# nadult/Snail

Measured on AMD Instinct MI355X. Metric: Mrays/sec (primary), higher is better.
Workload: dtype f32; 1 GPU; BASELINE config 1: atrium (263124 tris, sponza.obj stand-in) 1920x1080 primary rays, hit records (t,u,v,triId); reflections=False, arith=host_sse, arith_tables=host CPU, packets=16x16 px = 1 wavefront, bvh_nodes=161677, bvh_depth=21, frames_in_flight=16, frames_per_launch=4, launches_in_flight=4, settle_frames=332, order_refresh=16, ranks=1, packet_order=heaviest first (node visits of an earlier frame), parallelism=single-gpu

## Files before the change

include/snail_hip_debug.h:

```cpp
#ifndef SNAIL_HIP_DEBUG_H
#define SNAIL_HIP_DEBUG_H
#include "snail_hip.h"
#ifdef __cplusplus
extern "C" {
#endif

int snail_debug_delay_dev(float microseconds, void *stream);

int snail_debug_clock_dev(float microseconds, uint64_t *d_out2, void *stream);

int snail_debug_recip_check(uint64_t out2[2]);

int snail_debug_hostsse_device_check(int fn, int threads, uint64_t *badChunks, uint32_t *firstBadChunk);

int snail_debug_dispatch_rate(int blocks, int threads, int reps, float *ms_per_launch);

int snail_debug_anyorder(SnailScene *, const float cam[13], int resx, int resy, int frames, int flags, float *ms_total);

int snail_debug_occupancy(int out[4]);

#ifdef __cplusplus
}
#endif
#endif
```

snail_amd/_lib.py:

```python
from __future__ import annotations

import ctypes as C
import os

HERE = os.path.dirname(os.path.abspath(__file__))
LIB_PATH = os.environ.get("SNAIL_LIB_PATH") or os.path.join(HERE, "libsnailhip.so")


class SnailError(RuntimeError):
    pass


_lib = None

_VP, _I, _F13 = C.c_void_p, C.c_int, C.c_void_p
SIGNATURES = {
    "snail_last_error": (C.c_char_p, []),
    "snail_device_count": (_I, []),
    "snail_tris_from_verts": (_I, [_VP, _I, _VP]),
    "snail_bvh_build": (_I, [_VP, _I, _VP, _VP, _VP, _VP]),
    "snail_scene_create": (_VP, [_VP, _I, _VP, _I, _I, _I]),
    "snail_scene_destroy": (None, [_VP]),
    "snail_scene_info": (_I, [_VP, _VP, _VP, _VP, _VP]),
    "snail_scene_flags": (_I, [_VP, _VP, _VP]),
# ... 61 lines not shown
    "snail_instances_render_whitted_dev": (_I, [_VP, _F13, _I, _I, _VP, _I, _VP, _VP, _I, _VP, _I, _VP, _VP]),
    "snail_instances_render_whitted_packets_dev": (_I, [_VP, _F13, _I, _I, _VP, _I, _VP, _I, _VP, _VP, _I, _VP, _VP, _VP]),
    "snail_instances_render_image": (_I, [_VP, _F13, _I, _I, _VP, _I, _VP, _VP, _I, _VP, _I, _VP]),
}

INSTANCES_TILES_SIGNATURES = {
    "snail_instances_shade_packets_dev": (_I, [_VP, _F13, _I, _I, _VP, _I, _VP, _I, _VP, _VP, _I, _VP, _VP, _VP, _VP]),
    "snail_instances_render_tiles": (_I, [_VP, _F13, _I, _I, _VP, _VP, _I, _VP, _I, _VP, _VP, _I, _VP, _VP, _VP]),
    "snail_instances_render_frame": (_I, [_VP, _F13, _I, _I, _VP, _I, _VP, _VP, _I, _VP, _I, _VP]),
}

INSTANCES_BUILD_SIGNATURES = {
    "snail_instances_rebuild_dev": (_I, [_VP, _VP, _VP, _I, _VP, _VP, _VP]),
    "snail_instances_read_tree": (_I, [_VP, _VP, _I, _VP, _VP, _VP, _I, _VP]),
}

BVH_FAST_SIGNATURES = {
    "snail_bvh_build_fast": (_I, [_VP, _I, _VP, _VP, _VP, _VP]),
    "snail_scene_create_fast_dev": (_VP, [_VP, _I, _I, _VP, _VP, _VP]),
    "snail_scene_rebuild_fast_dev": (_I, [_VP, _VP, _I, _VP, _VP, _VP]),
}

HEATMAP_SIGNATURES = {
    "snail_packet_stats_dev": (_I, [_VP, _F13, _I, _I, _VP, _I, _VP, _I, _I, _VP, _VP, _VP]),
    "snail_render_heat_packets_dev": (_I, [_VP, _F13, _I, _I, _VP, _I, _VP, _I, _I, _VP, _VP, _VP, _VP]),
    "snail_render_heat_tiles": (_I, [_VP, _F13, _I, _I, _VP, _VP, _I, _VP, _I, _I, _VP, _VP]),
    "snail_render_heat_image": (_I, [_VP, _F13, _I, _I, _VP, _I, _I, _VP, _I, _VP]),
    "snail_instances_packet_stats_dev": (_I, [_VP, _F13, _I, _I, _VP, _I, _VP, _I, _I, _VP, _VP, _VP]),
    "snail_instances_heat_packets_dev": (_I, [_VP, _F13, _I, _I, _VP, _I, _VP, _I, _I, _VP, _VP, _VP, _VP, _VP]),
    "snail_instances_render_heat_tiles": (_I, [_VP, _F13, _I, _I, _VP, _VP, _I, _VP, _I, _I, _VP, _VP, _VP]),
    "snail_instances_render_heat_frame": (_I, [_VP, _F13, _I, _I, _VP, _I, _I, _VP, _I, _VP]),
}

MATERIALS_SIGNATURES = {
    "snail_shtris_pack": (_I, [_VP, _VP, _VP, _VP, _I, _VP, _VP]),
    "snail_texture_size": (C.c_int64, [_I, _I, _VP]),
    "snail_texture_build": (_I, [_VP, _I, _I, _VP, C.c_int64, _VP]),
    "snail_materials_create": (_VP, [_VP, _VP, _I, _VP, _I, _VP, _I, _VP, _I]),
    "snail_materials_destroy": (None, [_VP]),
    "snail_materials_shade_packets_dev": (_I, [_VP, _F13, _I, _I, _VP, _I, _VP, _VP, _VP, _VP, _VP, _VP]),
    "snail_render_materials_dev": (_I, [_VP, _F13, _I, _I, _VP, _I, _VP, _I, _VP, _I, _VP, _VP]),
    "snail_render_materials_packets_dev": (_I, [_VP, _F13, _I, _I, _VP, _I, _VP, _I, _VP, _I, _VP, _VP, _VP]),
    "snail_render_materials_image": (_I, [_VP, _F13, _I, _I, _VP, _I, _VP, _I, _VP, _I, _VP]),
}

DEBUG_SIGNATURES = {
    "snail_debug_delay_dev": (_I, [C.c_float, _VP]),
    "snail_debug_clock_dev": (_I, [C.c_float, _VP, _VP]),
    "snail_debug_recip_check": (_I, [_VP]),
    "snail_debug_dispatch_rate": (_I, [_I, _I, _I, _VP]),
    "snail_debug_hostsse_device_check": (_I, [_I, _I, _VP, _VP]),
    "snail_debug_occupancy": (_I, [_VP]),
    "snail_debug_anyorder": (_I, [_VP, _F13, _I, _I, _I, _I, _VP]),
}
DEBUG_LIB_PATH = os.path.join(HERE, "libsnailhip_debug.so")
_dbg = None


def debug_lib():
    global _dbg
    if _dbg is None:
        if not os.path.exists(DEBUG_LIB_PATH):
            raise SnailError("workbench library %s is missing: `make -C snail_amd/csrc debug`" % DEBUG_LIB_PATH)
        L = C.CDLL(DEBUG_LIB_PATH)
        for table in (SIGNATURES, INSTANCES_SIGNATURES, INSTANCES_SHADE_SIGNATURES, INSTANCES_TILES_SIGNATURES, INSTANCES_BUILD_SIGNATURES, BVH_FAST_SIGNATURES, HEATMAP_SIGNATURES, MATERIALS_SIGNATURES, DEBUG_SIGNATURES):
            for name, (res, args) in table.items():
                fn = getattr(L, name)
                fn.restype = res
                fn.argtypes = args
        _dbg = L
    return _dbg


def lib():
    global _lib
    if _lib is None:
        if not os.path.exists(LIB_PATH):
            raise SnailError(
                "HIP extension %s is missing: run `python -c 'import __graft_entry__ as g; g.build()'` "
                "(or `make -C snail_amd/csrc`). There is no CPU fallback." % LIB_PATH)
        try:
            L = C.CDLL(LIB_PATH)
        except OSError as e:
            raise SnailError("cannot load %s: %s" % (LIB_PATH, e)) from e
        for table in (SIGNATURES, INSTANCES_SIGNATURES, INSTANCES_SHADE_SIGNATURES, INSTANCES_TILES_SIGNATURES, INSTANCES_BUILD_SIGNATURES, BVH_FAST_SIGNATURES, HEATMAP_SIGNATURES, MATERIALS_SIGNATURES):
            for name, (res, args) in table.items():
                fn = getattr(L, name)
                fn.restype = res
                fn.argtypes = args
        for name, (res, args) in DEBUG_SIGNATURES.items():
            fn = getattr(L, name, None)
            if fn is not None:
                fn.restype = res
                fn.argtypes = args
        _lib = L
    return _lib


def check(rc: int, what: str) -> None:
    if rc != 0:
        msg = lib().snail_last_error()
        raise SnailError("%s failed (status %d): %s" % (what, rc, msg.decode() if msg else "?"))


def ptr(a):
    if a is None:
# ... 5 lines not shown
```

snail_amd/csrc/snail_dev.inc:

```
namespace SNAIL_DEV_NS {

typedef unsigned long long u64;
typedef unsigned u32x4 __attribute__((ext_vector_type(4)));
typedef const __attribute__((address_space(4))) u32x4 *scalar_ptr;

struct Node {
	float bmin[3], bmax[3];
	unsigned sub;
	int aux;
};

__device__ __forceinline__ float asf(unsigned u) { return __uint_as_float(u); }
__device__ __forceinline__ float asf(int u) { return __int_as_float(u); }

typedef const __attribute__((address_space(4))) char *scalar_bytes;
__device__ __forceinline__ Node loadNode(const uint4 *nodes, int idx) {
	const unsigned off = (unsigned)idx << 5;
	scalar_ptr p = (scalar_ptr)((scalar_bytes)(unsigned long long)nodes + off);
	u32x4 a = p[0], b = p[1];
	Node n;
	n.bmin[0] = asf(a.x); n.bmin[1] = asf(a.y); n.bmin[2] = asf(a.z);
	n.bmax[0] = asf(a.w); n.bmax[1] = asf(b.x); n.bmax[2] = asf(b.y);
	n.sub = b.z; n.aux = (int)b.w;
	return n;
// ... 875 lines not shown
	" v_readlane_b32 %[cur], %[stkN], %[sp]\n v_readlane_b32 %[fl], %[stkF], %[sp]\n"                                                      \
	" s_and_b32 %[first], %[fl], 0xff\n s_lshr_b32 %[last], %[fl], 8\n"
#define SNAIL_PUSH_2W                                                                                                                      \
	" s_lshl_b32 %[off], %[last], 8\n s_or_b32 %[off], %[off], %[first]\n"                                                                 \
	" s_mov_b32 m0, %[sp]\n v_writelane_b32 %[stkN], %[fl], m0\n v_writelane_b32 %[stkF], %[off], m0\n"
#define SNAIL_COUNT " s_add_u32 %[cnt], %[cnt], 1\n"
#define SNAIL_DRAIN_SMEM " s_waitcnt lgkmcnt(0)\n"
#define SNAIL_DESCEND_ASM(PRE, ORGOPS, SLAB, TAIL, CNTPOP, CNTVISIT, NX, FX, NY, FY, NZ, FZ)                                                 \
	asm volatile(SNAIL_DRAIN_SMEM                                                                                                          \
				 "L_pop_%=:\n"                                                                                                             \
				 " s_cmp_eq_u32 %[sp], 0\n s_cbranch_scc1 L_done_%=\n"                                                                     \
				 " s_sub_u32 %[sp], %[sp], 1\n" CNTPOP                                                                                     \
				 SNAIL_POP_2W                                                                                                              \
				 " s_lshl_b32 %[off], %[cur], 5\n s_load_dwordx8 s[84:91], %[base], %[off]\n"                                              \
				 " s_sub_u32 %[width], %[last], %[first]\n"                                                                                \
				 " s_bfm_b64 exec, %[width], %[first]\n s_bitset1_b64 exec, %[last]\n"                                                     \
				 " s_waitcnt lgkmcnt(0)\n"                                                                                                 \
				 "L_visit_%=:\n" CNTVISIT                                                                                                  \
				 PRE(NX, FX, NY, FY, NZ, FZ)                                                                                               \
				 SLAB("0", NX, FX, NY, FY, NZ, FZ) TAIL("0", "s0") SLAB("1", NX, FX, NY, FY, NZ, FZ) TAIL("1", "s1")                       \
				 SLAB("2", NX, FX, NY, FY, NZ, FZ) TAIL("2", "s2") SLAB("3", NX, FX, NY, FY, NZ, FZ) TAIL("3", "s3")                       \
				 " v_max_f32 %[s2], %[s2], %[s3]\n v_max3_f32 %[s0], %[s0], %[s1], %[s2]\n"                                                \
				 " v_cmp_le_f32 vcc, 0, %[s0]\n"                                                                                           \
				 " s_and_b64 %[alive], vcc, exec\n s_cbranch_scc0 L_pop_%=\n"                                                              \
				 " s_ff1_i32_b64 %[first], %[alive]\n s_flbit_i32_b64 %[last], %[alive]\n s_xor_b32 %[last], %[last], 63\n"                \
				 " s_sub_u32 %[width], %[last], %[first]\n"                                                                                \
				 " s_bfm_b64 exec, %[width], %[first]\n s_bitset1_b64 exec, %[last]\n"                                                     \
				 " s_cmp_lt_i32 s90, 0\n s_cbranch_scc1 L_leaf_%=\n"                                                                       \
				 " s_lshr_b32 %[cur], %[sign16], s91\n s_xor_b32 %[cur], %[cur], s91\n s_bfe_u32 %[cur], %[cur], 0x10010\n"                \
				 " s_add_u32 %[fl], s90, 1\n s_sub_u32 %[fl], %[fl], %[cur]\n"                                                             \
				 " s_add_u32 %[cur], s90, %[cur]\n s_lshl_b32 %[off], %[cur], 5\n"                                                         \
				 " s_load_dwordx8 s[84:91], %[base], %[off]\n"                                                                             \
				 SNAIL_PUSH_2W                                                                                                             \
				 " s_add_u32 %[sp], %[sp], 1\n"                                                                                            \
				 " s_waitcnt lgkmcnt(0)\n s_branch L_visit_%=\n"                                                                           \
				 "L_leaf_%=:\n s_mov_b32 %[leafSub], s90\n s_mov_b32 %[leafAux], s91\n s_branch L_end_%=\n"                                \
				 "L_done_%=:\n s_mov_b32 %[leafSub], 0\n s_mov_b32 %[leafAux], 0\n"                                                        \
				 "L_end_%=:\n s_mov_b64 exec, -1\n"                                                                                        \
				 : [sp] "+s"(sp), [first] "+s"(first), [last] "+s"(last), [cnt] "+s"(cnt), [stkN] "+v"(stkN), [stkF] "+v"(stkF),           \
				   [leafSub] "=&s"(leafSub), [leafAux] "=&s"(leafAux), [cur] "=&s"(sCur), [fl] "=&s"(sFl), [off] "=&s"(sOff),              \
				   [width] "=&s"(sWidth), [rng] "=&s"(sRng), [alive] "=&s"(sAlive), [pnx] "=&v"(vt[0]), [pny] "=&v"(vt[1]),                \
				   [pnz] "=&v"(vt[2]), [pfx] "=&v"(vt[3]), [pfy] "=&v"(vt[4]), [pfz] "=&v"(vt[5]), [t0] "=&v"(vt[6]), [t1] "=&v"(vt[7]),   \
				   [t2] "=&v"(vt[8]), [t3] "=&v"(vt[9]), [t4] "=&v"(vt[10]), [t5] "=&v"(vt[11]), [s0] "=&v"(vt[12]), [s1] "=&v"(vt[13]),   \
				   [s2] "=&v"(vt[14]), [s3] "=&v"(vt[15]), [u0] "=&v"(vt[16])                                                              \
				 : [base] "s"(nodeBase), [sign16] "s"(sign16), [lane] "v"(lane), ORGOPS(), [ix0] "v"(Q.id[0][0]), [ix1] "v"(Q.id[0][1]), [ix2] "v"(Q.id[0][2]), [ix3] "v"(Q.id[0][3]),        \
				   [iy0] "v"(Q.id[1][0]), [iy1] "v"(Q.id[1][1]), [iy2] "v"(Q.id[1][2]), [iy3] "v"(Q.id[1][3]), [iz0] "v"(Q.id[2][0]),      \
				   [iz1] "v"(Q.id[2][1]), [iz2] "v"(Q.id[2][2]), [iz3] "v"(Q.id[2][3]), [d0] "v"(Q.dist[0]), [d1] "v"(Q.dist[1]),          \
				   [d2] "v"(Q.dist[2]), [d3] "v"(Q.dist[3])                                                                                \
				 : "s84", "s85", "s86", "s87", "s88", "s89", "s90", "s91", "vcc", "scc", "m0");                                            \
	              \
	asm volatile("" ::"s"(sp), "s"(first), "s"(last), "s"(cnt), "v"(stkN), "v"(stkF), "s"(leafSub), "s"(leafAux), "s"(sCur), "s"(sFl), "s"(sOff),    \
				 "s"(sWidth), "s"(sRng), "s"(sAlive), "v"(vt[0]), "v"(vt[1]), "v"(vt[2]), "v"(vt[3]), "v"(vt[4]), "v"(vt[5]), "v"(vt[6]), "v"(vt[7]), \
				 "v"(vt[8]), "v"(vt[9]), "v"(vt[10]), "v"(vt[11]), "v"(vt[12]), "v"(vt[13]), "v"(vt[14]), "v"(vt[15]), "v"(vt[16]))
#define SNAIL_MOV_REC(D0, D1, D2, D3, S0, S1, S2, S3)                                                                                       \
	" s_mov_b64 " D0 ", " S0 "\n s_mov_b64 " D1 ", " S1 "\n s_mov_b64 " D2 ", " S2 "\n s_mov_b64 " D3 ", " S3 "\n"
#define SNAIL_A_FROM_T SNAIL_MOV_REC("s[84:85]", "s[86:87]", "s[88:89]", "s[90:91]", "s[68:69]", "s[70:71]", "s[72:73]", "s[74:75]")
#define SNAIL_PF_LEAFREQ_TRI(OTHERSET) " s_bitset0_b32 %[cur], 31\n s_load_dwordx8 " OTHERSET ", %[base], %[cur]\n"
#define SNAIL_PF_LEAFREQ_SLOT0(OTHERSET) " s_max_i32 %[cur], %[cur], 0\n s_load_dwordx8 " OTHERSET ", %[base], %[cur]\n"

#define SNAIL_PF2_NEARFAR(SUB, AUX, FARX, OTHERSET, LEAFREQ)                                                                                          \
				 " s_and_b32 %[cur], " AUX ", %[sign16]\n s_cselect_b32 %[cur], 32, 0\n"                                                       \
				 " s_xor_b32 %[cur], " SUB ", %[cur]\n s_xor_b32 " FARX ", %[cur], 32\n"                                                       \
				 LEAFREQ(OTHERSET)
#define SNAIL_PF2_TAIL(X, SUB)  \
				 " v_max_f32 %[s2], %[s2], %[s3]\n v_max3_f32 %[s0], %[s0], %[s1], %[s2]\n"                                                \
				 " v_cmpx_le_f32 vcc, 0, %[s0]\n"                                                                                           \
				 " s_cbranch_execz L_fail_%=\n"                                                                                            \
				 " s_cbranch_scc1 L_leaf" X "_%=\n"
#define SNAIL_PF2_ISLEAF(SUB) " s_cmp_lt_i32 " SUB ", 0\n"
#define SNAIL_PF2_ALIVE " s_sub_u32 %[cur], %[last], %[first]\n s_bfm_b64 %[alive], %[cur], %[first]\n s_bitset1_b64 %[alive], %[last]\n"
#define SNAIL_PF2_FIRSTLAST " s_ff1_i32_b64 %[first], exec\n s_flbit_i32_b64 %[last], exec\n s_xor_b32 %[last], %[last], 63\n"
#define SNAIL_PF2_PENDING(X, OTHERSET, SUB, AUX, FARX, FARY, PRE, SLAB, TAIL, CNTVISIT, LEAFREQ, NX, FX, NY, FY, NZ, FZ)                                                   \
				 "L_visit" X "p_%=:\n"                                                                                                      \
				 " s_waitcnt lgkmcnt(0)\n"                                                 \
				 " s_load_dwordx8 s[68:75], %[base], " FARY "\n"                              \
				 CNTVISIT PRE(NX, FX, NY, FY, NZ, FZ)                                                                                        \
				 SLAB("0", NX, FX, NY, FY, NZ, FZ) TAIL("0", "s0")                                                                           \
				 SNAIL_PF2_NEARFAR(SUB, AUX, FARX, OTHERSET, LEAFREQ)                                                                        \
				 SLAB("1", NX, FX, NY, FY, NZ, FZ) TAIL("1", "s1")                                                                           \
				 SNAIL_PF2_FIRSTLAST                                                      \
				 " s_lshl_b32 %[off], %[last], 6\n s_or_b32 %[off], %[off], %[first]\n s_lshl_b32 %[off], %[off], 20\n"                    \
				 SNAIL_PF2_ALIVE                                                                                                            \
				 SLAB("2", NX, FX, NY, FY, NZ, FZ) TAIL("2", "s2")                                                                           \
				 " s_lshr_b32 %[topw], " FARY ", 5\n s_or_b32 %[topw], %[topw], %[off]\n"                                                    \
				 " v_writelane_b32 %[stkN], %[topw], m0\n s_add_u32 m0, m0, 1\n" SNAIL_PF2_ISLEAF(SUB)                                       \
				 SLAB("3", NX, FX, NY, FY, NZ, FZ) TAIL("3", "s3")                                                                           \
				 SNAIL_PF2_TAIL(X, SUB)
#define SNAIL_PF2_LEAF(X, SUB, AUX)                                                                                                         \
				 "L_leaf" X "_%=:\n" SNAIL_PF2_FIRSTLAST                                                                                    \
				 " s_bfe_u32 %[leafSub], " SUB ", 0x190006\n s_sub_u32 %[leafSub], %[leafSub], 0x80000\n s_bitset1_b32 %[leafSub], 31\n"   \
				 " s_mov_b32 %[leafAux], " AUX "\n s_waitcnt lgkmcnt(0)\n s_branch L_end_%=\n"
#define SNAIL_DESCEND_PF2X(EXTRACLOB, PREVARS, PRE, ORGOPS, SLAB, TAIL, CNTPOP, CNTVISIT, LEAFREQ, NXA, FXA, NYA, FYA, NZA, FZA, NXB, FXB, NYB, FYB, NZB, FZB)                                                  \
	asm volatile(SNAIL_DRAIN_SMEM " s_mov_b32 m0, %[sp]\n"                                                                                \
				 "L_entry_%=:\n"                                                                                                           \
				 " s_cmp_eq_u32 m0, 0\n s_cbranch_scc1 L_done_%=\n"                                                                     \
				 " s_sub_u32 %[off], m0, 1\n"                                                                                           \
				 " v_readlane_b32 %[topw], %[stkN], %[off]\n"                                                                              \
				 " s_and_b32 %[cur], %[topw], 0xfffff\n s_lshl_b32 %[off], %[cur], 5\n"                                                    \
				 " s_load_dwordx8 s[68:75], %[base], %[off]\n"                                                                             \
				 " s_bfe_u32 %[first], %[topw], 0x60014\n s_lshr_b32 %[last], %[topw], 26\n" SNAIL_PF2_ALIVE                               \
				 "L_pop_%=:\n"                             \
				 " s_sub_u32 m0, m0, 1\n" CNTPOP                                                                                     \
				 " s_mov_b64 exec, %[alive]\n"                                                                                             \
				 " s_waitcnt lgkmcnt(0)\n" SNAIL_A_FROM_T                                                                                  \
				                   \
				 " s_sub_u32 %[off], m0, 1\n s_max_i32 %[off], %[off], 0\n"   \
				 " v_readlane_b32 %[topw], %[stkN], %[off]\n"                                                                              \
				 CNTVISIT PRE(NXA, FXA, NYA, FYA, NZA, FZA)                                                                                 \
				 SLAB("0", NXA, FXA, NYA, FYA, NZA, FZA) TAIL("0", "s0")                                                          \
				 " s_and_b32 %[cur], %[topw], 0xfffff\n s_lshl_b32 %[off], %[cur], 5\n"                                                    \
				 " s_load_dwordx8 s[68:75], %[base], %[off]\n"                                                                             \
				 SLAB("1", NXA, FXA, NYA, FYA, NZA, FZA) TAIL("1", "s1")                                                          \
				 SNAIL_PF2_NEARFAR("s90", "s91", "%[fl]", "s[76:83]", LEAFREQ)                                                                       \
				 SLAB("2", NXA, FXA, NYA, FYA, NZA, FZA) TAIL("2", "s2")                                                          \
				 " s_bfe_u32 %[first], %[topw], 0x60014\n s_lshr_b32 %[last], %[topw], 26\n" SNAIL_PF2_ALIVE SNAIL_PF2_ISLEAF("s90")        \
				 SLAB("3", NXA, FXA, NYA, FYA, NZA, FZA) TAIL("3", "s3")                                                          \
				 SNAIL_PF2_TAIL("A", "s90")                                                                                                 \
				                                                                    \
				 SNAIL_PF2_PENDING("B", "s[84:91]", "s82", "s83", "%[width]", "%[fl]", PRE, SLAB, TAIL, CNTVISIT, LEAFREQ, NXB, FXB, NYB, FYB, NZB, FZB)                   \
				                                                                    \
				 SNAIL_PF2_PENDING("A", "s[76:83]", "s90", "s91", "%[fl]", "%[width]", PRE, SLAB, TAIL, CNTVISIT, LEAFREQ, NXA, FXA, NYA, FYA, NZA, FZA)                   \
				 " s_branch L_visitBp_%=\n"                                                                                                \
				 SNAIL_PF2_LEAF("A", "s90", "s91") SNAIL_PF2_LEAF("B", "s82", "s83")                                                       \
				 "L_fail_%=:\n"                                                                                                            \
				 " s_cmp_eq_u32 m0, 0\n s_cbranch_scc0 L_pop_%=\n"                                                                      \
				 "L_done_%=:\n s_mov_b32 %[leafSub], 0\n s_mov_b32 %[leafAux], 0\n s_waitcnt lgkmcnt(0)\n"                                  \
				 "L_end_%=:\n s_mov_b64 exec, -1\n s_mov_b32 %[sp], m0\n"                                                                                        \
				 : [sp] "+s"(sp), [first] "+s"(first), [last] "+s"(last), [cnt] "+s"(cnt), [stkN] "+v"(stkN), [stkF] "+v"(stkF),           \
				   [leafSub] "=&s"(leafSub), [leafAux] "=&s"(leafAux), [cur] "=&s"(sCur), [fl] "=&s"(sFl), [off] "=&s"(sOff),              \
				   [width] "=&s"(sWidth), [topw] "=&s"(sTopw), [alive] "=&s"(sAlive), PREVARS() [t0] "=&v"(vt[6]), [t1] "=&v"(vt[7]),   \
				   [t2] "=&v"(vt[8]), [t3] "=&v"(vt[9]), [t4] "=&v"(vt[10]), [t5] "=&v"(vt[11]), [s0] "=&v"(vt[12]), [s1] "=&v"(vt[13]),   \
				   [s2] "=&v"(vt[14]), [s3] "=&v"(vt[15]), [u0] "=&v"(vt[16])                                                              \
				 : [base] "s"(nodeBase), [sign16] "s"(sign16), [lane] "v"(lane), ORGOPS(), [ix0] "v"(Q.id[0][0]), [ix1] "v"(Q.id[0][1]), [ix2] "v"(Q.id[0][2]), [ix3] "v"(Q.id[0][3]),        \
				   [iy0] "v"(Q.id[1][0]), [iy1] "v"(Q.id[1][1]), [iy2] "v"(Q.id[1][2]), [iy3] "v"(Q.id[1][3]), [iz0] "v"(Q.id[2][0]),      \
				   [iz1] "v"(Q.id[2][1]), [iz2] "v"(Q.id[2][2]), [iz3] "v"(Q.id[2][3]), [d0] "v"(Q.dist[0]), [d1] "v"(Q.dist[1]),          \
				   [d2] "v"(Q.dist[2]), [d3] "v"(Q.dist[3])                                                                                \
				 : "s68", "s69", "s70", "s71", "s72", "s73", "s74", "s75", "s76", "s77", "s78", "s79", "s80", "s81", "s82", "s83", "s84", "s85", "s86", "s87", \
				   "s88", "s89", "s90", "s91", "vcc", "scc", "m0" EXTRACLOB);                                                                        \
	asm volatile("" ::"s"(sp), "s"(first), "s"(last), "s"(cnt), "v"(stkN), "v"(stkF), "s"(leafSub), "s"(leafAux), "s"(sCur), "s"(sFl), "s"(sOff),    \
				 "s"(sWidth), "s"(sTopw), "s"(sAlive), "v"(vt[6]), "v"(vt[7]), \
				 "v"(vt[8]), "v"(vt[9]), "v"(vt[10]), "v"(vt[11]), "v"(vt[12]), "v"(vt[13]), "v"(vt[14]), "v"(vt[15]), "v"(vt[16]))
#define SNAIL_PREVARS_SHARED() [pnx] "=&v"(vt[0]), [pny] "=&v"(vt[1]), [pnz] "=&v"(vt[2]), [pfx] "=&v"(vt[3]), [pfy] "=&v"(vt[4]), [pfz] "=&v"(vt[5]),
#define SNAIL_PREVARS_NONE() [pnx] "=&v"(vt[0]), [pny] "=&v"(vt[1]), [pnz] "=&v"(vt[2]), [pfx] "=&v"(vt[3]), [pfy] "=&v"(vt[4]), [pfz] "=&v"(vt[5]),
#define SNAIL_PREVARS_SNAIL_PRE_SHARED SNAIL_PREVARS_SHARED
#define SNAIL_PREVARS_SNAIL_PRE_NONE SNAIL_PREVARS_NONE
#define SNAIL_PREVARS_SNAIL_PRE_SEL SNAIL_PREVARS_NONE
#define SNAIL_PREVARS_EMPTY()
#define SNAIL_PRE_NONE_X(NX, FX, NY, FY, NZ, FZ) ""
#define SNAIL_PREVARS_SNAIL_PRE_NONE_X SNAIL_PREVARS_EMPTY
#define SNAIL_PREVARS_of(PRE) SNAIL_PREVARS_##PRE
#define SNAIL_DESCEND_PF2(PRE, ORGOPS, SLAB, TAIL, CNTPOP, CNTVISIT, LEAFREQ, NXA, FXA, NYA, FYA, NZA, FZA, NXB, FXB, NYB, FYB, NZB, FZB)                 \
	SNAIL_DESCEND_PF2X(, SNAIL_PREVARS_of(PRE), PRE, ORGOPS, SLAB, TAIL, CNTPOP, CNTVISIT, LEAFREQ, NXA, FXA, NYA, FYA, NZA, FZA, NXB, FXB, NYB, FYB, NZB, FZB)
#define SNAIL_PRE_SEL(NX, FX, NY, FY, NZ, FZ)                                                                                               \
				 " s_bitcmp1_b32 %[sign16], 8\n s_cselect_b32 s62, " FX ", " NX "\n s_cselect_b32 s65, " NX ", " FX "\n"                       \
				 " s_bitcmp1_b32 %[sign16], 9\n s_cselect_b32 s63, " FY ", " NY "\n s_cselect_b32 s66, " NY ", " FY "\n"                       \
				 " s_bitcmp1_b32 %[sign16], 10\n s_cselect_b32 s64, " FZ ", " NZ "\n s_cselect_b32 s67, " NZ ", " FZ "\n"
#define SNAIL_SLABO_SEL(L, NX, FX, NY, FY, NZ, FZ) SNAIL_SLABO_COH(L, "s62", "s65", "s63", "s66", "s64", "s67")
#define SNAIL_SEL_CLOB , "s62", "s63", "s64", "s65", "s66", "s67"
#define SNAIL_DESCEND_PF2_SEL(ORGOPS, SLAB, TAIL, CNTPOP, CNTVISIT, LEAFREQ)                                                                \
	SNAIL_DESCEND_PF2X(SNAIL_SEL_CLOB, SNAIL_PREVARS_NONE, SNAIL_PRE_SEL, ORGOPS, SLAB, TAIL, CNTPOP, CNTVISIT, LEAFREQ, "s84", "s87", "s85", "s88", "s86", "s89", "s76", "s79", "s77", "s80", "s78", "s81")
#define SNAIL_DESCEND_PF2_PLAIN(PRE, ORGOPS, SLAB, TAIL, CNTPOP, CNTVISIT, LEAFREQ) SNAIL_DESCEND_PF2(PRE, ORGOPS, SLAB, TAIL, CNTPOP, CNTVISIT, LEAFREQ, "s84", "s87", "s85", "s88", "s86", "s89", "s76", "s79", "s77", "s80", "s78", "s81")
#define SNAIL_DESCEND_PF2_OCT(PRE, ORGOPS, SLAB, TAIL, CNTPOP, CNTVISIT, LEAFREQ, OCT)                                                                                                    \
	switch(OCT) {                                                                                                                          \
	case 0: SNAIL_DESCEND_PF2(PRE, ORGOPS, SLAB, TAIL, CNTPOP, CNTVISIT, LEAFREQ, "s84", "s87", "s85", "s88", "s86", "s89", "s76", "s79", "s77", "s80", "s78", "s81"); break;            \
	case 1: SNAIL_DESCEND_PF2(PRE, ORGOPS, SLAB, TAIL, CNTPOP, CNTVISIT, LEAFREQ, "s87", "s84", "s85", "s88", "s86", "s89", "s79", "s76", "s77", "s80", "s78", "s81"); break;            \
	case 2: SNAIL_DESCEND_PF2(PRE, ORGOPS, SLAB, TAIL, CNTPOP, CNTVISIT, LEAFREQ, "s84", "s87", "s88", "s85", "s86", "s89", "s76", "s79", "s80", "s77", "s78", "s81"); break;            \
	case 3: SNAIL_DESCEND_PF2(PRE, ORGOPS, SLAB, TAIL, CNTPOP, CNTVISIT, LEAFREQ, "s87", "s84", "s88", "s85", "s86", "s89", "s79", "s76", "s80", "s77", "s78", "s81"); break;            \
	case 4: SNAIL_DESCEND_PF2(PRE, ORGOPS, SLAB, TAIL, CNTPOP, CNTVISIT, LEAFREQ, "s84", "s87", "s85", "s88", "s89", "s86", "s76", "s79", "s77", "s80", "s81", "s78"); break;            \
	case 5: SNAIL_DESCEND_PF2(PRE, ORGOPS, SLAB, TAIL, CNTPOP, CNTVISIT, LEAFREQ, "s87", "s84", "s85", "s88", "s89", "s86", "s79", "s76", "s77", "s80", "s81", "s78"); break;            \
	case 6: SNAIL_DESCEND_PF2(PRE, ORGOPS, SLAB, TAIL, CNTPOP, CNTVISIT, LEAFREQ, "s84", "s87", "s88", "s85", "s89", "s86", "s76", "s79", "s80", "s77", "s81", "s78"); break;            \
	default: SNAIL_DESCEND_PF2(PRE, ORGOPS, SLAB, TAIL, CNTPOP, CNTVISIT, LEAFREQ, "s87", "s84", "s88", "s85", "s89", "s86", "s79", "s76", "s80", "s77", "s81", "s78"); break;           \
	}

#define SNAIL_DESCEND_OCT(PRE, ORGOPS, SLAB, TAIL, CNTPOP, CNTVISIT, OCT)                                                                     \
	switch(OCT) {                                                                                                                          \
	case 0: SNAIL_DESCEND_ASM(PRE, ORGOPS, SLAB, TAIL, CNTPOP, CNTVISIT, "s84", "s87", "s85", "s88", "s86", "s89"); break;                              \
// ... 1461 lines not shown
		const int xx = T.x + tx, yy = T.y + ty;
		if(xx >= resx || yy >= resy) continue;
		const unsigned char red = p[i];
		unsigned char *d = frame + (size_t)yy * pitch + (size_t)xx * 3;
		d[2] = red; d[1] = (unsigned char)(p[(size_t)n + i] + red); d[0] = (unsigned char)(p[(size_t)2 * n + i] + red);
	}
}

#ifdef SNAIL_DEBUG_API
__global__ __launch_bounds__(64) void k_delay(unsigned ticks) {
	const u64 t0 = __builtin_amdgcn_s_memrealtime();
	while((unsigned)(__builtin_amdgcn_s_memrealtime() - t0) < ticks) __builtin_amdgcn_s_sleep(1);
}

__global__ __launch_bounds__(64) void k_clock(unsigned ticks, unsigned long long *out) {
	const u64 r0 = __builtin_amdgcn_s_memrealtime(), c0 = __builtin_amdgcn_s_memtime();
	while((unsigned)(__builtin_amdgcn_s_memrealtime() - r0) < ticks) __builtin_amdgcn_s_sleep(1);
	const u64 c1 = __builtin_amdgcn_s_memtime(), r1 = __builtin_amdgcn_s_memrealtime();
	if(threadIdx.x == 0) { out[0] = c1 - c0; out[1] = r1 - r0; }
}

__global__ __launch_bounds__(256) void k_recip_check(unsigned base, unsigned long long *out) {
	const unsigned bits = base + blockIdx.x * 256u + threadIdx.x;
	const float x = __uint_as_float(bits);
	const float ref = 1.0f / x, got = recipExact(x);
	const bool same = (ref != ref) ? (got != got) : __float_as_uint(ref) == __float_as_uint(got);
	const bool inside = ((bits & 0x7f800000u) - 0x00800000u) < 0x7e000000u;
	const u64 bad = __builtin_amdgcn_ballot_w64(!same), in = __builtin_amdgcn_ballot_w64(inside);
	if((threadIdx.x & 63) == 0) {
		if(bad) atomicAdd(&out[0], (unsigned long long)__builtin_popcountll(bad));
		if(in) atomicAdd(&out[1], (unsigned long long)__builtin_popcountll(in));
	}
}

__global__ void k_nop(int *sink) { if(sink && threadIdx.x == 0 && blockIdx.x == 0x7fffffff) *sink = 1; }
#endif

__host__ __device__ inline void pfEncode(const unsigned (&in)[8], unsigned (&out)[8], unsigned trisOff) {
	for(int k = 0; k < 6; k++) out[k] = in[k];
	if(in[6] & 0x80000000u) { out[6] = 0x80000000u | (trisOff + ((in[6] & 0x7fffffffu) << 6)); out[7] = in[7]; }
	else { out[6] = (in[6] + 1u + (in[7] >> 16)) << 5; out[7] = 1u << (in[7] & 3u); }
}
__global__ __launch_bounds__(256) void k_pf_encode(const uint4 *__restrict__ nodes, int nNodes, unsigned trisOff, uint4 *__restrict__ pf) {
	const int i = (int)(blockIdx.x * 256 + threadIdx.x);
	if(i >= nNodes) return;
	const uint4 a = nodes[(size_t)i * 2], b = nodes[(size_t)i * 2 + 1];
	const unsigned in[8] = {a.x, a.y, a.z, a.w, b.x, b.y, b.z, b.w};
	unsigned out[8];
	pfEncode(in, out, trisOff);
	pf[(size_t)(i + 1) * 2] = make_uint4(out[0], out[1], out[2], out[3]);
	pf[(size_t)(i + 1) * 2 + 1] = make_uint4(out[4], out[5], out[6], out[7]);
}

__global__ __launch_bounds__(256) void k_rel_nodes(const uint4 *__restrict__ pf, int nSlots, float ox, float oy, float oz, uint4 *__restrict__ rel) {
	const int i = (int)(blockIdx.x * 256 + threadIdx.x);
	if(i >= nSlots) return;
	const uint4 a = pf[(size_t)i * 2], b = pf[(size_t)i * 2 + 1];
	const float o[3] = {ox, oy, oz};
	const unsigned in[6] = {a.x, a.y, a.z, a.w, b.x, b.y};
	unsigned out[6];
	for(int k = 0; k < 6; k++) out[k] = __float_as_uint(__uint_as_float(in[k]) - o[k % 3]);
	rel[(size_t)i * 2] = make_uint4(out[0], out[1], out[2], out[3]);
	rel[(size_t)i * 2 + 1] = make_uint4(out[4], out[5], b.z, b.w);
}

struct RelFillArgs {
	int n;
	float org[SNAIL_MAX_BATCH][3];
	uint4 *dst[SNAIL_MAX_BATCH];
};
__global__ __launch_bounds__(256) void k_rel_nodes_multi(const uint4 *__restrict__ pf, int nSlots, RelFillArgs A) {
	const int i = (int)(blockIdx.x * 256 + threadIdx.x);
	if(i >= nSlots) return;
	const uint4 a = pf[(size_t)i * 2], b = pf[(size_t)i * 2 + 1];
	const unsigned in[6] = {a.x, a.y, a.z, a.w, b.x, b.y};
	for(int f = 0; f < A.n; f++) {
		unsigned out[6];
		for(int k = 0; k < 6; k++) out[k] = __float_as_uint(__uint_as_float(in[k]) - A.org[f][k % 3]);
		A.dst[f][(size_t)i * 2] = make_uint4(out[0], out[1], out[2], out[3]);
		A.dst[f][(size_t)i * 2 + 1] = make_uint4(out[4], out[5], b.z, b.w);
	}
}

struct AccountArgs {
	const uint4 *nodes, *tris;
	GenConst g;
	int x0, y0, pw, ph;
	u64 *out;
};
__global__ __launch_bounds__(256) void k_account(AccountArgs A) {
	const int lane = threadIdx.x & 63;
	const int p = (int)blockIdx.x * 4 + (int)(threadIdx.x >> 6);
	if(p >= A.pw * A.ph) return;
	const int px = A.x0 + (p % A.pw) * 16, py = A.y0 + (p / A.pw) * 16;
	const int ty = lane >> 2, k4 = lane & 3;
	const float inf = __builtin_inff();
	unsigned vn = 0, vt = 0, hits = 0;
	for(int l = 0; l < 4; l++) {
		const float xoff = (float)(px + (l >= 2 ? 2 : 0)), yoff = (float)(py - (l >= 2 ? 1 : 0));
		const float tposx = (float)(4 * k4) + xoff, tposy = (float)ty + yoff;
		float pp[3], d[3], id[3];
		for(int c = 0; c < 3; c++) pp[c] = A.g.tright[c] * tposx + (A.g.tup[c] * tposy + A.g.txyz[c][l]);
		const float rs = 1.0f / __builtin_sqrtf(pp[0] * pp[0] + pp[1] * pp[1] + pp[2] * pp[2]);
		for(int c = 0; c < 3; c++) { d[c] = pp[c] * rs; id[c] = 1.0f / (d[c] + 0.00000001f); }
		const int sg[3] = {d[0] < 0.0f, d[1] < 0.0f, d[2] < 0.0f};
		int stack[SNAIL_MAX_DEPTH + 2], sp = 0;
		stack[sp++] = 0;
		float dist = inf;
		while(sp) {
			int cur = stack[--sp];
			for(;;) {
				const uint4 *np = A.nodes + (size_t)cur * 2;
				const uint4 a = np[0], b = np[1];
				const float bmin[3] = {asf(a.x), asf(a.y), asf(a.z)}, bmax[3] = {asf(a.w), asf(b.x), asf(b.y)};
				vn++;
				float lmin = 0.0f, lmax = 0.0f;
				for(int k = 0; k < 3; k++) {
					float l1 = id[k] * (bmin[k] - A.g.org[k]), l2 = id[k] * (bmax[k] - A.g.org[k]);
					float lo = Min<M_EXACT>(l1, l2), hi = Max<M_EXACT>(l1, l2);
					if(k == 0) { lmin = lo; lmax = hi; }
					else { lmin = Max<M_EXACT>(lmin, lo); lmax = Min<M_EXACT>(lmax, hi); }
				}
				if(lmax < 0.0f || lmin > Min<M_EXACT>(lmax, dist)) break;
				if(b.z & 0x80000000u) {
					const int count = (int)b.w, firstTri = (int)(b.z & 0x7fffffffu);
					for(int k = 0; k < count; k++) {
						const Tri t = loadTriVector(A.tris, firstTri + k);
						vt++;
						float tv[3] = {A.g.org[0] - t.a[0], A.g.org[1] - t.a[1], A.g.org[2] - t.a[2]};
						float t0v[3] = {(t.ba[1] * tv[2] - t.ba[2] * tv[1]) * t.it0, (t.ba[2] * tv[0] - t.ba[0] * tv[2]) * t.it0,
										(t.ba[0] * tv[1] - t.ba[1] * tv[0]) * t.it0};
						float t1v[3] = {(tv[1] * t.ca[2] - tv[2] * t.ca[1]) * t.it0, (tv[2] * t.ca[0] - tv[0] * t.ca[2]) * t.it0,
										(tv[0] * t.ca[1] - tv[1] * t.ca[0]) * t.it0};
						const float tmul = -(tv[0] * t.n[0] + tv[1] * t.n[1] + tv[2] * t.n[2]);
						const float det = d[0] * t.n[0] + d[1] * t.n[1] + d[2] * t.n[2];
// ... 27 lines not shown
```

snail_amd/csrc/snail_hip.hip:

```cpp
#include <hip/hip_runtime.h>
#include <hip/hip_ext.h>

#include <cmath>
#include <cstdarg>
#include <cstdio>
#include <algorithm>
#include <cstring>
#include <memory>
#include <mutex>
#include <utility>
#include <vector>

#include "../../include/snail_hip.h"
#include "../../include/snail_instances.h"
#include "../../include/snail_bvh_fast.h"
#include "host_sse.h"
#ifdef SNAIL_DEBUG_API
#include "../../include/snail_hip_debug.h"
#endif

static thread_local char g_err[1024] = "";

void snail_set_error(const char *fmt, ...) {
	va_list ap;
// ... 1471 lines not shown
}

int snail_debug_anyorder(SnailScene *s, const float cam[13], int resx, int resy, int frames, int flags, float *ms_total) {
	if(int rc = checkScene(s, "snail_debug_anyorder")) return rc;
	if(frames <= 0 || !ms_total || useDeep(s)) { snail_set_error("snail_debug_anyorder: bad arguments"); return 1; }
	DeviceGuard guard(s->device);
	dev::PrimaryArgs A;
	memset(&A, 0, sizeof(A));
	A.hostTab = nullptr;
	A.nodes = s->dNodes; A.tris = s->dTris; A.pf = (const uint4 *)s->dPF;
	A.nFrames = 1;
	A.g[0] = makeGen(cam, resx, resy);
	A.resx = resx; A.resy = resy; A.w = resx; A.h = resy;
	A.fastOK = s->fastOK && originSane(cam);
	A.pack = stackPack(s);
	A.pw = (resx + 15) / 16; A.ph = (resy + 15) / 16; A.nPackets = A.pw * A.ph;
	const int nRegions = ((A.pw + 3) / 4) * ((A.ph + 3) / 4);
	const int blocks = ((nRegions + 7) / 8) * 8 * 16;
	A.nBlocks = blocks; A.nSlots = blocks;
	if(blocks + 2 > s->deferCap) { snail_set_error("snail_debug_anyorder: trace one ordinary frame of this size first"); return 1; }
	A.defer = s->dDefer[0];
	hipStream_t st;
	HIP_TRY(hipStreamCreateWithFlags(&st, hipStreamNonBlocking));
	int relWhich = -1;
	if(A.pack && !useDeep(s)) {
		if(int rc = relFor(s, cam, st, &A.rel[0], &relWhich)) return rc;
	}
	hipEvent_t e0, e1;
	HIP_TRY(hipEventCreate(&e0)); HIP_TRY(hipEventCreate(&e1));
	HIP_TRY(hipDeviceSynchronize());
	HIP_TRY(hipEventRecord(e0, st));
	for(int f = 0; f < frames; f++)
		hipExtLaunchKernelGGL(dev::k_primary<false>, dim3(blocks), dim3(64), 0, st, nullptr, nullptr, (unsigned)flags, A);
	HIP_TRY(hipGetLastError());
	HIP_TRY(hipEventRecord(e1, st));
	HIP_TRY(hipStreamSynchronize(st));
	HIP_TRY(hipEventElapsedTime(ms_total, e0, e1));
	(void)hipEventDestroy(e0); (void)hipEventDestroy(e1); (void)hipStreamDestroy(st);
	return 0;
}

int snail_debug_occupancy(int out[4]) {
	if(!out) { snail_set_error("snail_debug_occupancy: null output"); return 1; }
	int dev = 0;
	HIP_TRY(hipGetDevice(&dev));
	int perCU = 0, maxBlocks = 0, cus = 0;
	HIP_TRY(hipOccupancyMaxActiveBlocksPerMultiprocessor(&perCU, (const void *)dev::k_primary<false>, 64, 0));
	HIP_TRY(hipDeviceGetAttribute(&maxBlocks, hipDeviceAttributeMaxBlocksPerMultiProcessor, dev));
	HIP_TRY(hipDeviceGetAttribute(&cus, hipDeviceAttributeMultiprocessorCount, dev));
	out[0] = perCU; out[1] = maxBlocks; out[2] = cus; out[3] = 1;
	return 0;
}

#endif

int snail_account_packets(SnailScene *s, const float cam[13], int resx, int resy, uint32_t *out8) {
	if(int rc = checkScene(s, "snail_account_packets")) return rc;
	if(!out8 || resx <= 0 || resy <= 0) { snail_set_error("snail_account_packets: null output or bad resolution"); return 1; }
	DeviceGuard guard(s->device);
	HostCallScope hc(s, "snail_account_packets");
	if(hc.rc) return hc.rc;
	const size_t bytes = (size_t)((resx + 15) / 16) * ((resy + 15) / 16) * 32;
	if(int rc = hc.reserve(HostCallScope::pad(bytes))) return rc;
	void *c = hc.carve(bytes);
	HIP_TRY(hipMemsetAsync(c, 0, bytes, hc.stream()));
	{
		SNAIL_LOCK(s);
		if(int rc = launchPrimary(s, cam, resx, resy, 0, 0, resx, resy, nullptr, 0, nullptr, nullptr, nullptr, nullptr, nullptr, hc.stream(), (unsigned *)c)) return rc;
	}
	if(int rc = hc.get(out8, c, bytes)) return rc;
	return hc.finish(nullptr);
}

int snail_account_primary(SnailScene *s, const float cam[13], int resx, int resy, int x0, int y0, int w, int h, uint64_t out[4]) {
	if(int rc = checkScene(s, "snail_account_primary")) return rc;
	if((x0 & 15) || (y0 & 15) || w <= 0 || h <= 0 || !out) { snail_set_error("snail_account_primary: bad rect"); return 1; }
	DeviceGuard guard(s->device);
	HostCallScope hc(s, "snail_account_primary");
	if(hc.rc) return hc.rc;
	dev::AccountArgs A;
	A.nodes = s->dNodes; A.tris = s->dTris;
	A.g = makeGen(cam, resx, resy);
	A.x0 = x0; A.y0 = y0; A.pw = (w + 15) / 16; A.ph = (h + 15) / 16;
	A.out = (dev::u64 *)hc.stats();
	if(int rc = hc.zeroStats()) return rc;
	const int np = A.pw * A.ph;
	{
		SNAIL_LOCK(s);
		SceneUse use(s, hc.stream());
		if(use.rc) return use.rc;
		hipLaunchKernelGGL(dev::k_account, dim3((np + 3) / 4), dim3(256), 0, hc.stream(), A);
		HIP_TRY(hipGetLastError());
	}
	return hc.finish(out);
}

}

#include "bvh_fast.inc"
#include "render_host.inc"
#include "instances_host.inc"
#include "instances_tiles_host.inc"
#include "heatmap_host.inc"
#include "materials_host.inc"
```

Baseline: 26960 Mrays/s.

## Flag BVH nodes containing the ray origin and skip their slab test

When building the origin-relative node copies, each inner node whose box contains the shared ray origin gets bit 31 of its aux word set. The packet traversal assembly tests that bit before the slab test and jumps to new copies of the descent code that push the far child without doing box intersection. For primary rays from a common camera origin, every ray hits such boxes, so the slab arithmetic can be skipped on those nodes. It adds code size, an extra scalar test and branch on every visit, and a debug kernel that counts the flagged nodes.

```diff
diff --git a/include/snail_hip_debug.h b/include/snail_hip_debug.h
--- a/include/snail_hip_debug.h
+++ b/include/snail_hip_debug.h
@@ -19,6 +19,8 @@
 
 int snail_debug_occupancy(int out[4]);
 
+int snail_debug_rel_flag_count(SnailScene *, const float org[3], int *count);
+
 #ifdef __cplusplus
 }
 #endif
diff --git a/snail_amd/_lib.py b/snail_amd/_lib.py
--- a/snail_amd/_lib.py
+++ b/snail_amd/_lib.py
@@ -137,6 +137,7 @@
     "snail_debug_hostsse_device_check": (_I, [_I, _I, _VP, _VP]),
     "snail_debug_occupancy": (_I, [_VP]),
     "snail_debug_anyorder": (_I, [_VP, _F13, _I, _I, _I, _I, _VP]),
+    "snail_debug_rel_flag_count": (_I, [_VP, _VP, _VP]),
 }
 DEBUG_LIB_PATH = os.path.join(HERE, "libsnailhip_debug.so")
 _dbg = None
diff --git a/snail_amd/csrc/snail_dev.inc b/snail_amd/csrc/snail_dev.inc
--- a/snail_amd/csrc/snail_dev.inc
+++ b/snail_amd/csrc/snail_dev.inc
@@ -951,6 +951,7 @@
 	asm volatile("" ::"s"(sp), "s"(first), "s"(last), "s"(cnt), "v"(stkN), "v"(stkF), "s"(leafSub), "s"(leafAux), "s"(sCur), "s"(sFl), "s"(sOff),    \
 				 "s"(sWidth), "s"(sRng), "s"(sAlive), "v"(vt[0]), "v"(vt[1]), "v"(vt[2]), "v"(vt[3]), "v"(vt[4]), "v"(vt[5]), "v"(vt[6]), "v"(vt[7]), \
 				 "v"(vt[8]), "v"(vt[9]), "v"(vt[10]), "v"(vt[11]), "v"(vt[12]), "v"(vt[13]), "v"(vt[14]), "v"(vt[15]), "v"(vt[16]))
+#define SNAIL_REL_INSIDE_BIT 31
 #define SNAIL_MOV_REC(D0, D1, D2, D3, S0, S1, S2, S3)                                                                                       \
 	" s_mov_b64 " D0 ", " S0 "\n s_mov_b64 " D1 ", " S1 "\n s_mov_b64 " D2 ", " S2 "\n s_mov_b64 " D3 ", " S3 "\n"
 #define SNAIL_A_FROM_T SNAIL_MOV_REC("s[84:85]", "s[86:87]", "s[88:89]", "s[90:91]", "s[68:69]", "s[70:71]", "s[72:73]", "s[74:75]")
@@ -969,10 +970,35 @@
 #define SNAIL_PF2_ISLEAF(SUB) " s_cmp_lt_i32 " SUB ", 0\n"
 #define SNAIL_PF2_ALIVE " s_sub_u32 %[cur], %[last], %[first]\n s_bfm_b64 %[alive], %[cur], %[first]\n s_bitset1_b64 %[alive], %[last]\n"
 #define SNAIL_PF2_FIRSTLAST " s_ff1_i32_b64 %[first], exec\n s_flbit_i32_b64 %[last], exec\n s_xor_b32 %[last], %[last], 63\n"
+static_assert(SNAIL_REL_INSIDE_BIT == 31, "SNAIL_OIN_TEST_SNAIL_TAIL_POS names the bit in its text");
+#define SNAIL_OIN_TEST_SNAIL_TAIL_POS(AUX, LBL) " s_bitcmp1_b32 " AUX ", 31\n s_cbranch_scc1 " LBL "_%=\n"
+#define SNAIL_OIN_TEST_SNAIL_TAIL_ANY(AUX, LBL) ""
+#define SNAIL_OIN_TEST_of(TAIL) SNAIL_OIN_TEST_##TAIL
+#define SNAIL_OIN_PENDING(X, Y, OTHERSET, SUB, AUX, FARX, FARY, CNTVISIT, LEAFREQ)                                                          \
+				 "L_oin" X "p_%=:\n" CNTVISIT                                          \
+				 SNAIL_PF2_NEARFAR(SUB, AUX, FARX, OTHERSET, LEAFREQ)                                                                        \
+				 SNAIL_PF2_FIRSTLAST                                                           \
+				 " s_lshl_b32 %[off], %[last], 6\n s_or_b32 %[off], %[off], %[first]\n s_lshl_b32 %[off], %[off], 20\n"                    \
+				 SNAIL_PF2_ALIVE                                                                                                            \
+				 " s_lshr_b32 %[topw], " FARY ", 5\n s_or_b32 %[topw], %[topw], %[off]\n"                                                    \
+				 " v_writelane_b32 %[stkN], %[topw], m0\n s_add_u32 m0, m0, 1\n"                                                            \
+				 " s_branch L_visit" Y "p_%=\n"
+#define SNAIL_OIN_COPIES_SNAIL_TAIL_POS(CNTVISIT, LEAFREQ)                                                                                  \
+				 "L_oinAq_%=:\n" CNTVISIT                                                 \
+				 " s_and_b32 %[cur], %[topw], 0xfffff\n s_lshl_b32 %[off], %[cur], 5\n"                                                    \
+				 " s_load_dwordx8 s[68:75], %[base], %[off]\n"                                                                             \
+				 SNAIL_PF2_NEARFAR("s90", "s91", "%[fl]", "s[76:83]", LEAFREQ)                                                               \
+				 " s_bfe_u32 %[first], %[topw], 0x60014\n s_lshr_b32 %[last], %[topw], 26\n" SNAIL_PF2_ALIVE                               \
+				 " s_branch L_visitBp_%=\n"                                                                                                \
+				 SNAIL_OIN_PENDING("B", "A", "s[84:91]", "s82", "s83", "%[width]", "%[fl]", CNTVISIT, LEAFREQ)                               \
+				 SNAIL_OIN_PENDING("A", "B", "s[76:83]", "s90", "s91", "%[fl]", "%[width]", CNTVISIT, LEAFREQ)
+#define SNAIL_OIN_COPIES_SNAIL_TAIL_ANY(CNTVISIT, LEAFREQ) ""
+#define SNAIL_OIN_COPIES_of(TAIL) SNAIL_OIN_COPIES_##TAIL
 #define SNAIL_PF2_PENDING(X, OTHERSET, SUB, AUX, FARX, FARY, PRE, SLAB, TAIL, CNTVISIT, LEAFREQ, NX, FX, NY, FY, NZ, FZ)                                                   \
 				 "L_visit" X "p_%=:\n"                                                                                                      \
 				 " s_waitcnt lgkmcnt(0)\n"                                                 \
 				 " s_load_dwordx8 s[68:75], %[base], " FARY "\n"                              \
+				 SNAIL_OIN_TEST_of(TAIL)(AUX, "L_oin" X "p")                                                                                  \
 				 CNTVISIT PRE(NX, FX, NY, FY, NZ, FZ)                                                                                        \
 				 SLAB("0", NX, FX, NY, FY, NZ, FZ) TAIL("0", "s0")                                                                           \
 				 SNAIL_PF2_NEARFAR(SUB, AUX, FARX, OTHERSET, LEAFREQ)                                                                        \
@@ -1005,6 +1031,7 @@
 				                   \
 				 " s_sub_u32 %[off], m0, 1\n s_max_i32 %[off], %[off], 0\n"   \
 				 " v_readlane_b32 %[topw], %[stkN], %[off]\n"                                                                              \
+				 SNAIL_OIN_TEST_of(TAIL)("s91", "L_oinAq")                                                                                  \
 				 CNTVISIT PRE(NXA, FXA, NYA, FYA, NZA, FZA)                                                                                 \
 				 SLAB("0", NXA, FXA, NYA, FYA, NZA, FZA) TAIL("0", "s0")                                                          \
 				 " s_and_b32 %[cur], %[topw], 0xfffff\n s_lshl_b32 %[off], %[cur], 5\n"                                                    \
@@ -1021,6 +1048,7 @@
 				 SNAIL_PF2_PENDING("A", "s[76:83]", "s90", "s91", "%[fl]", "%[width]", PRE, SLAB, TAIL, CNTVISIT, LEAFREQ, NXA, FXA, NYA, FYA, NZA, FZA)                   \
 				 " s_branch L_visitBp_%=\n"                                                                                                \
 				 SNAIL_PF2_LEAF("A", "s90", "s91") SNAIL_PF2_LEAF("B", "s82", "s83")                                                       \
+				 SNAIL_OIN_COPIES_of(TAIL)(CNTVISIT, LEAFREQ)                                                                               \
 				 "L_fail_%=:\n"                                                                                                            \
 				 " s_cmp_eq_u32 m0, 0\n s_cbranch_scc0 L_pop_%=\n"                                                                      \
 				 "L_done_%=:\n s_mov_b32 %[leafSub], 0\n s_mov_b32 %[leafAux], 0\n s_waitcnt lgkmcnt(0)\n"                                  \
@@ -2588,6 +2616,17 @@
 	pf[(size_t)(i + 1) * 2 + 1] = make_uint4(out[4], out[5], out[6], out[7]);
 }
 
+__host__ __device__ inline bool relOriginInside(const unsigned (&w)[6]) {
+	bool in = true;
+	for(int k = 0; k < 3; k++) {
+		const float n = __builtin_bit_cast(float, w[k]), f = __builtin_bit_cast(float, w[3 + k]);
+		in = in && n <= 0.0f && f >= 0.0f;
+	}
+	return in;
+}
+__host__ __device__ inline unsigned relAux(const unsigned (&rel)[6], unsigned sub, unsigned aux) {
+	return !(sub & 0x80000000u) && (aux & 7u) && relOriginInside(rel) ? aux | (1u << SNAIL_REL_INSIDE_BIT) : aux;
+}
 __global__ __launch_bounds__(256) void k_rel_nodes(const uint4 *__restrict__ pf, int nSlots, float ox, float oy, float oz, uint4 *__restrict__ rel) {
 	const int i = (int)(blockIdx.x * 256 + threadIdx.x);
 	if(i >= nSlots) return;
@@ -2597,7 +2636,7 @@
 	unsigned out[6];
 	for(int k = 0; k < 6; k++) out[k] = __float_as_uint(__uint_as_float(in[k]) - o[k % 3]);
 	rel[(size_t)i * 2] = make_uint4(out[0], out[1], out[2], out[3]);
-	rel[(size_t)i * 2 + 1] = make_uint4(out[4], out[5], b.z, b.w);
+	rel[(size_t)i * 2 + 1] = make_uint4(out[4], out[5], b.z, relAux(out, b.z, b.w));
 }
 
 struct RelFillArgs {
@@ -2614,9 +2653,17 @@
 		unsigned out[6];
 		for(int k = 0; k < 6; k++) out[k] = __float_as_uint(__uint_as_float(in[k]) - A.org[f][k % 3]);
 		A.dst[f][(size_t)i * 2] = make_uint4(out[0], out[1], out[2], out[3]);
-		A.dst[f][(size_t)i * 2 + 1] = make_uint4(out[4], out[5], b.z, b.w);
-	}
-}
+		A.dst[f][(size_t)i * 2 + 1] = make_uint4(out[4], out[5], b.z, relAux(out, b.z, b.w));
+	}
+}
+#ifdef SNAIL_DEBUG_API
+__global__ __launch_bounds__(256) void k_rel_flag_count(const uint4 *__restrict__ rel, int nSlots, unsigned long long *__restrict__ out) {
+	const int i = (int)(blockIdx.x * 256 + threadIdx.x);
+	const bool flagged = i < nSlots && !(rel[(size_t)i * 2 + 1].z & 0x80000000u) && ((rel[(size_t)i * 2 + 1].w >> SNAIL_REL_INSIDE_BIT) & 1u);
+	const u64 m = __builtin_amdgcn_ballot_w64(flagged);
+	if((threadIdx.x & 63) == 0 && m) atomicAdd(out, (unsigned long long)__builtin_popcountll(m));
+}
+#endif
 
 struct AccountArgs {
 	const uint4 *nodes, *tris;
diff --git a/snail_amd/csrc/snail_hip.hip b/snail_amd/csrc/snail_hip.hip
--- a/snail_amd/csrc/snail_hip.hip
+++ b/snail_amd/csrc/snail_hip.hip
@@ -1547,6 +1547,32 @@
 	return 0;
 }
 
+int snail_debug_rel_flag_count(SnailScene *s, const float org[3], int *count) {
+	if(int rc = checkScene(s, "snail_debug_rel_flag_count")) return rc;
+	if(!org || !count) { snail_set_error("snail_debug_rel_flag_count: null argument"); return 1; }
+	if(!stackPack(s)) { snail_set_error("snail_debug_rel_flag_count: this scene keeps no origin-relative node records"); return 1; }
+	DeviceGuard guard(s->device);
+	HostCallScope hc(s, "snail_debug_rel_flag_count");
+	if(hc.rc) return hc.rc;
+	if(int rc = hc.zeroStats()) return rc;
+	{
+		SNAIL_LOCK(s);
+		SceneUse use(s, hc.stream());
+		if(use.rc) return use.rc;
+		const uint4 *rel = nullptr;
+		int which = -1;
+		if(int rc = relFor(s, org, hc.stream(), &rel, &which)) return rc;
+		const int nSlots = s->nNodes + 1;
+		hipLaunchKernelGGL(dev::k_rel_flag_count, dim3((unsigned)((nSlots + 255) / 256)), dim3(256), 0, hc.stream(), rel, nSlots, (unsigned long long *)hc.stats());
+		HIP_TRY(hipGetLastError());
+		if(int rc = relUsed(s, which, hc.stream())) return rc;
+	}
+	uint64_t st[4] = {0, 0, 0, 0};
+	if(int rc = hc.finish(st)) return rc;
+	*count = (int)st[0];
+	return 0;
+}
+
 #endif
 
 int snail_account_packets(SnailScene *s, const float cam[13], int resx, int resy, uint32_t *out8) {
```

New measurement: 27380 Mrays/s (median of 6 runs). 1.02x the previous value.
